# ysymyth/3D-SDN

Hardware: AMD Instinct MI355X
Metric: rendered-objects/sec (FFD decode + transform + silhouette/normal/depth @384, fwd+bwd) (higher is better)
Workload: dtype f32

## Files before the change

3d-sdn_amd/csrc/fast_ffd.hip:

```cpp
#include "sdn_common.h"

namespace sdn {

constexpr int NCOEF_MAX = 512;

__global__ __launch_bounds__(256) void k_ffd_fwd(const float* __restrict__ Bt, const float* __restrict__ P,
                                                  const int32_t* __restrict__ cls, int vmax, int ncoef,
                                                  float* __restrict__ out)
{
    __shared__ float Ps[3 * NCOEF_MAX];
    const int b = blockIdx.y;
    for (int t = threadIdx.x; t < 3 * ncoef; t += 256) Ps[t] = P[(size_t)b * 3 * ncoef + t];
    __syncthreads();
    const int v = blockIdx.x * 256 + threadIdx.x;
    if (v >= vmax) return;
    const float* bt = Bt + (size_t)cls[b] * ncoef * vmax + v;
    float x = 0.f, y = 0.f, z = 0.f;
#pragma unroll 8
    for (int j = 0; j < ncoef; j++) {
        const float w = bt[(size_t)j * vmax];
        x += Ps[j] * w;
        y += Ps[ncoef + j] * w;
        z += Ps[2 * ncoef + j] * w;
    }
// ... 21 lines not shown
        const float g0 = gb[3 * v + 0], g1 = gb[3 * v + 1], g2 = gb[3 * v + 2];
#pragma unroll
        for (int u = 0; u < FFD_JB; u++) {
            const float w = (j0 + u < ncoef) ? bt[(size_t)u * vmax + v] : 0.f;
            s[u][0] += g0 * w;
            s[u][1] += g1 * w;
            s[u][2] += g2 * w;
        }
    }
#pragma unroll
    for (int u = 0; u < FFD_JB; u++) {
#pragma unroll
        for (int o = 32; o > 0; o >>= 1) {
            s[u][0] += __shfl_xor(s[u][0], o, 64);
            s[u][1] += __shfl_xor(s[u][1], o, 64);
            s[u][2] += __shfl_xor(s[u][2], o, 64);
        }
        if ((threadIdx.x & 63) == 0) {
            red[u][0][threadIdx.x >> 6] = s[u][0];
            red[u][1][threadIdx.x >> 6] = s[u][1];
            red[u][2][threadIdx.x >> 6] = s[u][2];
        }
    }
    __syncthreads();
    if (threadIdx.x < 3 * FFD_JB) {
        const int u = threadIdx.x / 3, d = threadIdx.x % 3;
        if (j0 + u < ncoef) {
            float t = 0.f;
#pragma unroll
            for (int w = 0; w < NW; w++) t += red[u][d][w];
            grad_P[((size_t)b * 3 + d) * ncoef + j0 + u] = t;
        }
    }
}

__global__ __launch_bounds__(256) void k_ffd_coefficients(const float* __restrict__ x, const float* __restrict__ M,
                                                          const float* __restrict__ base, int m, int transpose,
                                                          float* __restrict__ out)
{
    extern __shared__ float xrow[];
    float* part = xrow + m;
    const int i = blockIdx.y;
    for (int k = threadIdx.x; k < m; k += 256) xrow[k] = x[(size_t)i * m + k];
    __syncthreads();
    const int jj = threadIdx.x & 63, kq = threadIdx.x >> 6;
    const int j = blockIdx.x * 64 + jj;
    const int per = (m + 3) / 4, k0 = kq * per, k1 = min(m, k0 + per);
    float acc = 0.0f;
    if (j < m) {
        if (transpose) {
            const float* row = M + (size_t)j * m;
#pragma unroll 8
            for (int k = k0; k < k1; k++) acc = fmaf(xrow[k], row[k], acc);
        } else {
#pragma unroll 8
            for (int k = k0; k < k1; k++) acc = fmaf(xrow[k], M[(size_t)k * m + j], acc);
        }
    }
    part[kq * 64 + jj] = acc;
    __syncthreads();
    if (kq == 0 && j < m)
        out[(size_t)i * m + j] = (base ? base[j] : 0.0f) + ((part[jj] + part[64 + jj]) + (part[128 + jj] + part[192 + jj]));
}

}

using namespace sdn;

SDN_API int sdn_ffd_coefficients(const float* x, const float* M, const float* base, int n, int m, int transpose, float* out,
                                 sdnStream stream)
{
    if (!x || !M || !out || n <= 0 || m <= 0 || m > 12288)
        return fail(SDN_EINVAL, "sdn_ffd_coefficients: bad arguments (m <= 12288)");
    hipLaunchKernelGGL(k_ffd_coefficients, dim3(cdiv(m, 64), n), dim3(256), (size_t)(m + 256) * sizeof(float), (hipStream_t)stream,
                       x, M, base, m, transpose, out);
    return check_launch("k_ffd_coefficients");
}

SDN_API int sdn_ffd_decode(const float* Bt, const float* P, const int32_t* cls, int n, int vmax, int ncoef, float* out,
                           sdnStream stream)
{
    if (!Bt || !P || !cls || !out || n <= 0 || vmax <= 0 || ncoef <= 0 || ncoef > NCOEF_MAX)
        return fail(SDN_EINVAL, "sdn_ffd_decode: bad arguments (ncoef <= %d)", NCOEF_MAX);
    hipLaunchKernelGGL(k_ffd_fwd, dim3(cdiv(vmax, 256), n), dim3(256), 0, (hipStream_t)stream, Bt, P, cls, vmax, ncoef,
                       out);
    return check_launch("k_ffd_fwd");
}

SDN_API int sdn_ffd_decode_bwd(const float* Bt, const int32_t* cls, const float* grad_out, int n, int vmax, int ncoef,
                               float* grad_P, sdnStream stream)
{
    if (!Bt || !cls || !grad_out || !grad_P || n <= 0 || vmax <= 0 || ncoef <= 0 || ncoef > NCOEF_MAX)
        return fail(SDN_EINVAL, "sdn_ffd_decode_bwd: bad arguments");
    hipLaunchKernelGGL(k_ffd_bwd, dim3(cdiv(ncoef, FFD_JB), n), dim3(FFD_BWD_THREADS), 0, (hipStream_t)stream, Bt, cls, grad_out, vmax, ncoef,
                       grad_P);
    return check_launch("k_ffd_bwd");
}
```

3d-sdn_amd/geometric/derender3d/models/transforms.py:

```python
import numpy as np
import scipy.special
import torch

from torch.nn.modules import Module


class _Constraint(object):

    class Type:
        symmetry = 0
        homogeneity = 1

    class Axis:
        x = 0
        y = 1
        z = 2

    def __init__(self, type, axis=None, index=None):
        self.type = type
        self.axis = axis
        self.index = index

    @classmethod
    def symmetry(cls, axis):
# ... 25 lines not shown
            shape = [1] * dP.dim()
            shape[comp] = 3
            dP = dP.index_copy(ax, idx, torch.where(keep.reshape(shape), planes, mean))
    return dP


def bernstein_basis(t, one_minus_t, n):
    i = torch.arange(n, dtype=torch.float32)
    binom = torch.tensor(scipy.special.binom(n - 1, np.arange(n)), dtype=torch.float32)
    return binom * torch.pow(t[:, None], i) * torch.pow(one_minus_t[:, None], n - 1 - i)


class FFD(Module):

    Constraint = _Constraint

    @staticmethod
    def flip(x, dim):
        return torch.flip(x, dims=(dim,))

    def __init__(self, vertices, num_grids=4, constraints=None):
        super(FFD, self).__init__()
        if num_grids % 2:
            raise AssertionError('num_grids must be even')
        self.num_grids = num_grids
        self.constraints = list(constraints) if constraints is not None else []
        v = torch.as_tensor(vertices, dtype=torch.float32)
        per_axis = [bernstein_basis(0.5 + v[:, d], 0.5 - v[:, d], num_grids) for d in range(3)]
        B = torch.einsum('ni,nj,nk->nijk', per_axis[0], per_axis[1], per_axis[2])
        lattice = torch.linspace(0, num_grids - 1, num_grids)
        P0 = torch.stack(torch.meshgrid(lattice, lattice, lattice, indexing='ij')) / (num_grids - 1) - 0.5
        self.register_buffer('B', B[:, None], persistent=False)
        self.register_buffer('P0', P0, persistent=False)

    def constrain(self, ffd_coeff):
        g = self.num_grids
        return apply_constraints(ffd_coeff.reshape(3, g, g, g), self.constraints)

    def forward(self, ffd_coeff):
        dP = self.constrain(ffd_coeff)
        n3 = self.num_grids ** 3
        P = (self.P0.to(dP.device) + dP).reshape(3, n3)
        return torch.matmul(self.B.to(dP.device).reshape(-1, n3), P.t())


def constrain_batched(dP, constraints, num_grids):
    return apply_constraints(dP, constraints)


class FFDBank(Module):

    def __init__(self, ffds, faces_list):
        super(FFDBank, self).__init__()
        from sdn_hip import ops
        self.num_grids = ffds[0].num_grids
        self.constraints = ffds[0].constraints
        n3 = self.num_grids ** 3
        self.nverts = [int(f.B.shape[0]) for f in ffds]
        self.nfaces = [int(f.shape[0]) for f in faces_list]
        vmax, fmax = max(self.nverts), max(self.nfaces)
        Bt = torch.zeros(len(ffds), n3, vmax)
        faces = torch.zeros(len(ffds), fmax, 3, dtype=torch.int32)
        for c, (ffd, f) in enumerate(zip(ffds, faces_list)):
            B = ffd.B.reshape(-1, n3)
            Bt[c, :, :B.shape[0]] = B.t()
            Bt[c, :, B.shape[0]:] = B[0][:, None]
            faces[c, :f.shape[0]] = f
        self.register_buffer('Bt', Bt.contiguous(), persistent=False)
        self.register_buffer('faces', faces.contiguous(), persistent=False)
        self.register_buffer('P0', ffds[0].P0.reshape(3, n3).clone(), persistent=False)
        eye = torch.eye(3 * n3).reshape(3 * n3, 3, self.num_grids, self.num_grids, self.num_grids)
        C = constrain_batched(eye, self.constraints, self.num_grids).reshape(3 * n3, 3 * n3)
        self.register_buffer('constraint_matrix', C.contiguous(), persistent=False)

    def decode(self, ffd_coeffs, classes):
        from sdn_hip import ops
        n = ffd_coeffs.shape[0]
        g = self.num_grids
        cls, faces = self._class_rows(classes)
        verts = ops.FFDDecode.apply(ffd_coeffs.reshape(n, 3 * g ** 3), self.Bt, cls, self.constraint_matrix, self.P0)
        return verts, faces

    def _class_rows(self, classes):
        hit = self.__dict__.get('_rows_cache')
        if hit is not None and hit[0] is classes and hit[1] == classes._version:
            return hit[2], hit[3]
        cls = classes.to(torch.int32)
        faces = self.faces.index_select(0, classes.long())
        self.__dict__['_rows_cache'] = (classes, classes._version, cls, faces)
        return cls, faces


    def invalidate_class_cache(self):
        self.__dict__.pop('_rows_cache', None)


class PerspectiveTransform(Module):
    def forward(self,
                vertices,
                scales=None,
                rotations=None,
                translations=None,
                perspective_translations=None,
                zooms=None,
                zoom_tos=None):
        if (vertices.is_cuda and scales is not None and rotations is not None and translations is not None
                and (zoom_tos is None) != (zooms is None) and vertices.dim() == 3):
            from sdn_hip import ops
            n = vertices.shape[0]
            persp = translations if perspective_translations is None else perspective_translations

            def full(x, k):
                return x.reshape(-1, k).expand(n, k) if x.shape[0] != n else x.reshape(n, k)
            t3 = full(translations, 3)
# ... 37 lines not shown
```

3d-sdn_amd/sdn_hip/__init__.py:

```python
import ctypes
import os
import threading

import torch

_HERE = os.path.dirname(os.path.abspath(__file__))
LIB_PATH = os.path.normpath(os.path.join(_HERE, '..', 'lib', 'libsdn_hip.so'))

RGB, ALPHA, DEPTH, AA, FACE_COLOR, SAVE_MAPS, ACCUMULATE, SERIAL_EDGES, STREAM_FACES, COUNT_WORK = 1, 2, 4, 8, 16, 32, 64, 128, 256, 512
K1_COVERAGE = 4096

ABI_VERSION = 20

_lib = None
_lock = threading.Lock()
_vp = ctypes.c_void_p
_ci = ctypes.c_int
_cl = ctypes.c_long
_cd = ctypes.c_double
_sz = ctypes.c_size_t


class SdnHipError(RuntimeError):
    pass


def _declare(L):
    L.sdn_last_error.restype = ctypes.c_char_p
    L.sdn_version.restype = _ci
    sig = {
        'sdn_project_vertices': [_vp, _ci, _ci, _ci, _vp, _vp, _vp, _vp, _ci, _vp, _vp],
        'sdn_project_vertices_bwd': [_vp, _ci, _ci, _ci, _vp, _vp, _vp, _vp, _ci, _vp, _vp, _vp],
        'sdn_gather_faces': [_vp, _vp, _ci, _ci, _ci, _cl, _ci, _vp, _vp],
        'sdn_gather_faces_bwd': [_vp, _vp, _ci, _ci, _ci, _cl, _ci, _vp, _vp],
        'sdn_face_normals': [_vp, _cl, _vp, _vp],
        'sdn_face_normals_bwd': [_vp, _vp, _cl, _vp, _vp],
        'sdn_raster_workspace_bytes': [_ci, _ci, _ci, ctypes.POINTER(_sz)],
        'sdn_rasterize_fwd': [_vp, _vp, _ci, _ci, _ci, _ci, _cd, _cd, _cd, _vp, _ci, _ci, _vp, _vp, _vp, _vp, _vp,
                              _vp, _vp, _vp, _vp, _sz, _vp],
        'sdn_raster_bwd_workspace_bytes': [_ci, _ci, _ci, ctypes.POINTER(_sz)],
        'sdn_rasterize_bwd': [_vp, _vp, _ci, _ci, _ci, _ci, _cd, _ci, _vp, _vp, _vp, _vp, _vp, _vp, _vp, _vp, _vp,
                              _vp, _vp, _sz, _vp],
    }
    sig['sdn_raster_work_counters'] = [_vp, _ci, _ci, _ci, ctypes.POINTER(ctypes.c_ulonglong), _vp]
    sig['sdn_ffd_decode'] = [_vp, _vp, _vp, _ci, _ci, _ci, _vp, _vp]
    sig['sdn_ffd_decode_bwd'] = [_vp, _vp, _vp, _ci, _ci, _ci, _vp, _vp]
    _i8p = ctypes.POINTER(ctypes.c_int8)
    _cf = ctypes.c_float
    sig['sdn_conv_gemm_workspace_bytes'] = [_ci, _ci, _ci, _ci, ctypes.POINTER(_sz)]
    sig['sdn_conv_gemm'] = [_vp, _ci, _ci, _ci, _ci, _vp, _ci, _ci, _ci, _ci, _ci, _ci, _ci, _ci, _ci, _ci, _i8p, _i8p,
                            _ci, _ci, _vp, _ci, _ci, _vp, _ci, _vp, _ci, _ci, _vp, _sz, _vp]
    _i32p = ctypes.POINTER(ctypes.c_int32)
    sig['sdn_conv_gemm_phases'] = [_vp, _ci, _ci, _ci, _ci, _vp, _ci, _ci, _ci, _ci, _ci, _ci, _i32p, _i32p, _i32p, _i32p, _i32p, _i8p,
                                   _ci, _ci, ctypes.POINTER(_vp), _i32p, _ci, _vp, _ci, _vp, _ci, _ci, _vp]
    sig['sdn_conv_wgrad'] = [_vp, _vp, _vp, _ci, _ci, _ci, _ci, _ci, _ci, _ci, _ci, _ci, _i8p, _i8p, _ci, _ci, _ci, _ci,
                             _ci, _vp, _sz, _vp]
    sig['sdn_conv_wgrad_narrow'] = [_vp, _vp, _vp, _ci, _ci, _ci, _ci, _ci, _ci, _ci, _ci, _ci, _i8p, _i8p, _ci, _ci, _ci,
                                    _vp]
    sig['sdn_conv_wgrad_head_mfma'] = [_vp, _vp, _vp, _ci, _ci, _ci, _ci, _ci, _ci, _ci, _ci, _ci, _i8p, _i8p, _ci, _ci, _ci,
                                    _vp]
    sig['sdn_conv_narrow_fwd'] = [_vp, _ci, _ci, _ci, _ci, _vp, _ci, _ci, _ci, _ci, _vp, _ci, _ci, _ci, _ci, _ci, _ci,
                                  _vp, _ci, _vp]
    sig['sdn_conv_head_steps'] = [_ci, _ci, _ci, ctypes.POINTER(_ci)]
    sig['sdn_conv_head_mfma'] = [_vp, _ci, _ci, _ci, _ci, _vp, _ci, _ci, _ci, _ci, _vp, _ci, _ci, _ci, _ci, _ci, _ci, _vp, _ci, _vp, _vp]
    sig['sdn_in_apply'] = [_vp, _vp, _vp, _vp, _vp, _ci, _ci, _ci, _ci, _cf, _ci, _ci, _cf, _vp, _vp, _vp, _cl, _ci, _vp]
    sig['sdn_in_bwd'] = [_vp, _vp, _vp, _vp, _ci, _ci, _ci, _ci, _vp, _cl, _vp]
    sig['sdn_act_bwd'] = [_vp, _vp, _vp, _cl, _ci, _ci, _vp, _cl, _vp]
    sig['sdn_reflect_fold'] = [_vp, _vp, _ci, _ci, _ci, _ci, _ci, _ci, _vp]
    sig['sdn_conv_pack_weights'] = [_vp, _ci, _ci, _cl, _cl, _vp, _ci, _ci, _ci, _ci, _vp, _vp]
    sig['sdn_conv_unpack_grad'] = [_vp, _ci, _ci, _cl, _cl, _vp, _ci, _ci, _vp, _ci, _vp]
    sig['sdn_split_planes'] = [_vp, _cl, _ci, _vp, _cl, _vp]
    sig['sdn_assemble_nhwc'] = [_vp, _vp, _ci, _ci, _ci, _ci, _ci, _vp, _vp]
    sig['sdn_conv_pack_weights_kmajor'] = [_vp, _ci, _ci, _cl, _cl, _vp, _ci, _ci, _ci, _vp, _vp]
    sig['sdn_conv_tile'] = [_vp, _cl, _ci, _ci, _ci, _ci, _vp, _vp, _cl, _ci, _ci, _ci, _ci, _ci, _ci, _ci, _ci, _ci, _ci, _ci,
                            _i8p, _i8p, _ci, _vp, _ci, _vp, _ci, _vp, _ci, _ci, _vp]
    sig['sdn_conv_halo_blocks'] = [_ci, _ci, _ci, _ci, _ci, _ci, ctypes.POINTER(_ci), ctypes.POINTER(_ci), ctypes.POINTER(_cl)]
    sig['sdn_conv_halo'] = [_vp, _cl, _ci, _ci, _ci, _ci, _vp, _ci, _ci, _ci, _ci, _i8p, _i8p, _ci, _vp, _ci, _vp, _ci, _vp, _ci, _vp]
    sig['sdn_conv_wgrad_tile'] = [_vp, _cl, _vp, _cl, _vp, _ci, _ci, _ci, _ci, _ci, _ci, _ci, _ci, _ci, _i8p, _i8p, _ci, _vp]
    sig['sdn_segment_mean'] = [_vp, _vp, _ci, _ci, _ci, _ci, _vp, _vp, _vp, _vp]
# ... 91 lines not shown
    for name, argtypes in sig.items():
        try:
            fn = getattr(L, name)
        except AttributeError:
            raise SdnHipError('%s does not export %s -- rebuild it (`python __graft_entry__.py build`)' % (LIB_PATH, name))
        fn.argtypes = argtypes
        fn.restype = _ci
    return sig


def lib():
    global _lib
    if _lib is None:
        with _lock:
            if _lib is None:
                if not os.path.exists(LIB_PATH):
                    raise SdnHipError(
                        'libsdn_hip.so not found at %s -- run `python __graft_entry__.py build` (hipcc, gfx950); '
                        'there is no CPU or PyTorch fallback for this path' % LIB_PATH)
                L = ctypes.CDLL(LIB_PATH)
                L.sdn_version.restype = _ci
                have = L.sdn_version()
                if have != ABI_VERSION:
                    raise SdnHipError('%s reports ABI version %d, this binding needs %d -- rebuild it '
                                      '(`python __graft_entry__.py build`)' % (LIB_PATH, have, ABI_VERSION))
                _declare(L)
                _lib = L
    return _lib


def exported_symbols():
    return ['sdn_last_error', 'sdn_version', 'sdn_project_vertices', 'sdn_project_vertices_bwd', 'sdn_gather_faces',
            'sdn_gather_faces_bwd', 'sdn_face_normals', 'sdn_face_normals_bwd', 'sdn_raster_workspace_bytes',
            'sdn_rasterize_fwd', 'sdn_raster_work_counters', 'sdn_raster_bwd_workspace_bytes', 'sdn_rasterize_bwd', 'sdn_ffd_decode', 'sdn_ffd_decode_bwd', 'sdn_ffd_coefficients',
            'sdn_timing_enable', 'sdn_timing_declare_work', 'sdn_timing_read', 'sdn_timing_read_slot', 'sdn_conv_gemm', 'sdn_conv_gemm_phases', 'sdn_conv_gemm_workspace_bytes', 'sdn_conv_wgrad', 'sdn_conv_wgrad_narrow', 'sdn_conv_wgrad_head_mfma', 'sdn_conv_narrow_fwd', 'sdn_conv_head_steps', 'sdn_conv_head_mfma', 'sdn_in_apply', 'sdn_in_bwd',
            'sdn_act_bwd', 'sdn_reflect_fold', 'sdn_conv_pack_weights', 'sdn_conv_unpack_grad', 'sdn_split_planes', 'sdn_conv_pack_weights_kmajor',
            'sdn_conv_tile', 'sdn_conv_wgrad_tile', 'sdn_conv_halo', 'sdn_conv_halo_blocks', 'sdn_segment_mean', 'sdn_l1_loss_fwd', 'sdn_l1_loss_bwd', 'sdn_silhouette_loss_fwd', 'sdn_silhouette_loss_bwd', 'sdn_assemble_nhwc', 'sdn_pose_params', 'sdn_pose_algebra', 'sdn_pose_algebra_bwd',
            'sdn_pose_params_bwd', 'sdn_composite_frame', 'sdn_edit_assemble', 'sdn_scene_cover', 'sdn_scene_crops', 'sdn_scene_edit',
            'sdn_unmold_masks', 'sdn_scene_gt_masks', 'sdn_scene_paint2d',
            'sdn_scene_id_workspace_bytes', 'sdn_scene_id_stats', 'sdn_scene_id_planes', 'sdn_assemble_planes', 'sdn_assemble_maps',
            'sdn_train_rois', 'sdn_train_crops', 'sdn_train_id_stats_workspace_bytes', 'sdn_train_id_stats', 'sdn_train_crops_mixed',
            'sdn_train_losses_scratch', 'sdn_train_losses_fwd', 'sdn_train_losses_bwd',
            'sdn_segm_fuse', 'sdn_segm_labels_from_colors', 'sdn_segm_confusion', 'sdn_segm_train_batch', 'sdn_segm_loss_fwd', 'sdn_segm_loss_bwd',
            'sdn_segm_ppm_pool', 'sdn_segm_ppm_fill', 'sdn_segm_ppm_fill_bwd', 'sdn_segm_ppm_pool_bwd',
            'sdn_encode_maps', 'sdn_inst_index_workspace_bytes', 'sdn_inst_index_build', 'sdn_inst_index_rank',
            'sdn_mrcnn_loss_workspace_bytes', 'sdn_mrcnn_loss_fwd', 'sdn_mrcnn_loss_bwd',
            'sdn_pyramid_roi_align_grad_floats', 'sdn_pyramid_roi_align_fwd', 'sdn_pyramid_roi_align_bwd',
            'sdn_proposal_layer_workspace_bytes', 'sdn_proposal_layer',
            'sdn_detection_layer_workspace_bytes', 'sdn_detection_layer',
            'sdn_detection_targets_workspace_bytes', 'sdn_detection_targets',
            'sdn_rpn_targets_workspace_bytes', 'sdn_rpn_targets',
            'sdn_perspective_transform_scratch', 'sdn_perspective_transform', 'sdn_perspective_transform_bwd', 'sdn_bn_forward', 'sdn_bn_backward',
            'sdn_maxpool3x3s2_fwd', 'sdn_maxpool3x3s2_bwd', 'sdn_avgpool_global', 'sdn_nms_workspace_bytes', 'sdn_nms',
            'sdn_crop_and_resize_fwd', 'sdn_crop_and_resize_bwd', 'sdn_avgpool3x3s2_fwd', 'sdn_avgpool3x3s2_bwd', 'sdn_render_maps_bytes', 'sdn_render_maps_fwd', 'sdn_raster_phase_clocks',
            'sdn_render_maps_bwd', 'sdn_program_create', 'sdn_program_run',
            'sdn_program_destroy']


def check(rc):
    if rc != 0:
        raise SdnHipError('libsdn_hip error %d: %s' % (rc, lib().sdn_last_error().decode()))


def ptr(t):
    return None if t is None else t.data_ptr()


# ... 10 lines not shown
        raise NotImplementedError('%s is on %s; this renderer only runs on the GPU' % (name, t.device))
    if t.dtype != dtype:
        raise TypeError('%s must be %s, got %s' % (name, dtype, t.dtype))
    return t.contiguous()


_const_cache = {}


def const_f32(values, device):
    import numpy as np
    a = np.ascontiguousarray(np.asarray(values, dtype=np.float32))
    key = (a.tobytes(), a.shape, str(device))
    t = _const_cache.get(key)
    if t is None:
        if len(_const_cache) > 4096:
            _const_cache.clear()
        t = _const_cache[key] = torch.tensor(a, device=device)
    return t


def raster_workspace(bs, nf, S, device):
    n = _sz(0)
    check(lib().sdn_raster_workspace_bytes(bs, nf, S, ctypes.byref(n)))
    return torch.empty(n.value, dtype=torch.uint8, device=device)


def perspective_transform_scratch(n, V):
    kb, ab = _sz(0), _sz(0)
    check(lib().sdn_perspective_transform_scratch(n, V, ctypes.byref(kb), ctypes.byref(ab)))
    return kb.value, ab.value


def train_losses_scratch(B, R, nffd):
    n = _sz(0)
    check(lib().sdn_train_losses_scratch(B, R, nffd, ctypes.byref(n)))
    return n.value


def raster_bwd_workspace(bs, nf, S, device):
    n = _sz(0)
    check(lib().sdn_raster_bwd_workspace_bytes(bs, nf, S, ctypes.byref(n)))
    return torch.empty(n.value, dtype=torch.uint8, device=device)


def scene_id_workspace(device):
    n = _sz(0)
    check(lib().sdn_scene_id_workspace_bytes(ctypes.byref(n)))
    return torch.empty(n.value, dtype=torch.uint8, device=device)


def train_id_workspace(B, device):
    n = _sz(0)
    check(lib().sdn_train_id_stats_workspace_bytes(int(B), ctypes.byref(n)))
    return torch.empty(n.value, dtype=torch.uint8, device=device)


def timing_enable(on=True):
    check(lib().sdn_timing_enable(int(bool(on))))


def timing_read():
    ms, n = _cd(0), _cl(0)
    check(lib().sdn_timing_read(ctypes.byref(ms), ctypes.byref(n)))
    return ms.value, n.value

# ... 10 lines not shown
```

3d-sdn_amd/sdn_hip/ops.py:

```python
import ctypes

import numpy as np
import torch
from torch.autograd.function import once_differentiable

from . import (AA, ACCUMULATE, ALPHA, COUNT_WORK, DEPTH, FACE_COLOR, K1_COVERAGE, RGB, SAVE_MAPS, SERIAL_EDGES, STREAM_FACES, check, lib, ptr, raster_bwd_workspace,
               raster_workspace, scene_id_workspace, stream, train_id_workspace, want)

CAMERA_NONE, CAMERA_LOOK, CAMERA_LOOK_AT = 0, 1, 2

import threading

_tls = threading.local()


class verification:

    def __init__(self, serial_edges=None, stream_faces=None, count_work=None):
        new = dict(serial_edges=serial_edges, stream_faces=stream_faces, count_work=count_work)
        self.new = {k: v for k, v in new.items() if v is not None}

    def __enter__(self):
        self.old = {k: getattr(_tls, k, False) for k in self.new}
        for k, v in self.new.items():
# ... 21 lines not shown
    return _K1[0]


def last_clocks():
    return getattr(_tls, 'last_clocks', None)


def last_work():
    return getattr(_tls, 'last_work', None)


def perspective_width(angle):
    a = np.float32(angle)
    a = np.float32(a / np.float32(180.))
    a = np.float32(a * np.float32(3.1416))
    return np.float32(np.tan(a, dtype=np.float32))


def _f32(t, name):
    return want(t, torch.float32, name)


_ptf_sizes = {}


def _ptf_scratch(n, V):
    r = _ptf_sizes.get((n, V))
    if r is None:
        from . import perspective_transform_scratch
        if len(_ptf_sizes) > 256:
            _ptf_sizes.clear()
        r = _ptf_sizes[(n, V)] = perspective_transform_scratch(n, V)
    return r


class ProjectVertices(torch.autograd.Function):
    @staticmethod
    def forward(ctx, vertices, camera_mode, eye, direction, up, width, flip_x):
        v = _f32(vertices, 'vertices')
        if v.dim() != 3 or v.shape[2] != 3:
            raise ValueError('vertices must be [batch, n, 3]')
        bs, nv = v.shape[:2]
        eye = _f32(eye, 'eye')
        direction = _f32(direction, 'direction')
        up = _f32(up, 'up')
        width = _f32(width, 'width')
        for t, n in ((eye, 'eye'), (direction, 'direction'), (up, 'up')):
            if t is not None and tuple(t.shape) != (bs, 3):
                raise ValueError('%s must be [batch, 3]' % n)
        if width is not None and width.numel() != bs:
            raise ValueError('width must have one entry per batch element')
        out = torch.empty_like(v)
        check(lib().sdn_project_vertices(ptr(v), bs, nv, int(camera_mode), ptr(eye), ptr(direction), ptr(up),
                                         ptr(width), int(flip_x), ptr(out), stream()))
        ctx.save_for_backward(v, eye, direction, up, width)
        ctx.cfg = (int(camera_mode), int(flip_x))
        return out

    @staticmethod
    def backward(ctx, g):
        v, eye, direction, up, width = ctx.saved_tensors
        mode, flip_x = ctx.cfg
        g = g.contiguous()
        gv = torch.empty_like(v)
        bs, nv = v.shape[:2]
        check(lib().sdn_project_vertices_bwd(ptr(v), bs, nv, mode, ptr(eye), ptr(direction), ptr(up), ptr(width),
# ... 225 lines not shown
                ctx.save_for_backward(v, f, state, cam[1], cam[2], cam[3], cam[4], bg)
                ctx.bg = None
            else:
                ctx.save_for_backward(v, f, state, cam[1], cam[2], cam[3], cam[4])
                ctx.bg = bg
            ctx.cfg = (bs, nv, nf0, stride, int(bool(fill_back)), cam[0], cam[5], R, flags & ~STREAM_FACES, float(eps),
                       float(eps_alpha), nbwd.value, SERIAL_EDGES if _switch('serial_edges') else 0)
        ctx.set_materialize_grads(False)
        return alpha, normal, depth

    @staticmethod
    def backward(ctx, g_alpha, g_normal, g_depth):
        saved = ctx.saved_tensors
        v, f, state, eye, direction, up, width = saved[:7]
        bg = saved[7] if len(saved) > 7 else ctx.bg
        bs, nv, nf0, stride, fill_back, mode, flip_x, R, flags, eps, eps_alpha, nbwd, serial = ctx.cfg
        if g_alpha is None and g_normal is None and g_depth is None:
            return (None,) * 18
        g_alpha = None if g_alpha is None else g_alpha.contiguous()
        g_normal = None if g_normal is None else g_normal.contiguous()
        g_depth = None if g_depth is None else g_depth.contiguous()
        ws = torch.empty(nbwd, dtype=torch.uint8, device=v.device)
        gv = torch.empty_like(v)
        check(lib().sdn_render_maps_bwd(ptr(v), bs, nv, ptr(f), nf0, stride, fill_back, mode, ptr(eye), ptr(direction), ptr(up),
                                        ptr(width), flip_x, R, flags | serial, eps, eps_alpha, ptr(bg), ptr(g_alpha),
                                        ptr(g_normal), ptr(g_depth), ptr(gv), ptr(state), state.numel(), ptr(ws), ws.numel(),
                                        stream()))
        return (gv,) + (None,) * 17


class FFDDecode(torch.autograd.Function):

    @staticmethod
    def forward(ctx, P, Bt, cls, constraint=None, base=None):
        P = _f32(P, 'P')
        Bt = _f32(Bt, 'Bt')
        cls = want(cls, torch.int32, 'cls')
        n = P.shape[0]
        ncoef = Bt.shape[1] if Bt.dim() == 3 else -1
        if constraint is not None:
            Cm = _f32(constraint, 'constraint')
            m = 3 * ncoef
            if P.dim() != 2 or P.shape[1] != m or tuple(Cm.shape) != (m, m) or (base is not None and base.numel() != m):
                raise ValueError('FFDDecode: coefficients [n, 3 ncoef], constraint [3 ncoef, 3 ncoef], base [3, ncoef]')
            base = None if base is None else _f32(base, 'base')
            coeffs = P
            P = torch.empty((n, 3, ncoef), dtype=torch.float32, device=coeffs.device)
            check(lib().sdn_ffd_coefficients(ptr(coeffs), ptr(Cm), ptr(base), n, m, 0, ptr(P), stream()))
        else:
            Cm = None
        if P.dim() != 3 or P.shape[1] != 3 or Bt.dim() != 3 or P.shape[2] != ncoef or cls.numel() != n:
            raise ValueError('FFDDecode: P [n,3,ncoef], Bt [classes,ncoef,vmax], cls [n]')
        vmax = Bt.shape[2]
        out = torch.empty((n, vmax, 3), dtype=torch.float32, device=P.device)
        check(lib().sdn_ffd_decode(ptr(Bt), ptr(P), ptr(cls), n, vmax, ncoef, ptr(out), stream()))
        if Cm is None:
            ctx.save_for_backward(Bt, cls)
        else:
            ctx.save_for_backward(Bt, cls, Cm)
        ctx.cfg = (n, vmax, ncoef)
        return out

    @staticmethod
    def backward(ctx, g):
        Bt, cls = ctx.saved_tensors[:2]
        n, vmax, ncoef = ctx.cfg
        g = g.contiguous()
        gP = torch.empty((n, 3, ncoef), dtype=torch.float32, device=g.device)
        check(lib().sdn_ffd_decode_bwd(ptr(Bt), ptr(cls), ptr(g), n, vmax, ncoef, ptr(gP), stream()))
        if len(ctx.saved_tensors) == 3:
            gc = torch.empty((n, 3 * ncoef), dtype=torch.float32, device=g.device)
            check(lib().sdn_ffd_coefficients(ptr(gP), ptr(ctx.saved_tensors[2]), None, n, 3 * ncoef, 1, ptr(gc), stream()))
            return gc, None, None, None, None
        return gP, None, None, None, None


class PoseParamsFn(torch.autograd.Function):

    @staticmethod
    def forward(ctx, theta, log_scales):
        th = _f32(theta, 'theta').reshape(-1)
        n = th.shape[0]
        ls = _f32(log_scales, 'log_scales').reshape(n, 3)
        quat = torch.empty(n, 4, dtype=torch.float32, device=th.device)
        scales = torch.empty(n, 3, dtype=torch.float32, device=th.device)
        check(lib().sdn_pose_params(ptr(th), ptr(ls), n, ptr(quat), ptr(scales), stream()))
        ctx.save_for_backward(th, scales)
        ctx.shapes = (theta.shape, log_scales.shape)
        ctx.set_materialize_grads(False)
        return quat, scales

    @staticmethod
    def backward(ctx, g_quat, g_scales):
        th, scales = ctx.saved_tensors
        n = th.shape[0]
        want_t, want_s = ctx.needs_input_grad
        if g_quat is None and g_scales is None:
            return None, None
        gq = g_quat.contiguous() if g_quat is not None else None
        gs = g_scales.contiguous() if g_scales is not None else None
        gt = torch.empty(n, dtype=torch.float32, device=th.device) if want_t else None
        gl = torch.empty(n, 3, dtype=torch.float32, device=th.device) if want_s else None
        if gt is None and gl is None:
            return None, None
        check(lib().sdn_pose_params_bwd(ptr(th), ptr(scales), ptr(gq), ptr(gs), n, ptr(gt), ptr(gl), stream()))
        return (gt.reshape(ctx.shapes[0]) if gt is not None else None, gl.reshape(ctx.shapes[1]) if gl is not None else None)

# ... 1665 lines not shown
```

include/sdn_hip.h:

```cpp
#ifndef SDN_HIP_H
#define SDN_HIP_H

#include <stddef.h>
#include <stdint.h>

#ifdef __cplusplus
extern "C" {
#endif

typedef void* sdnStream;

#define SDN_OK 0
#define SDN_EINVAL (-1)
#define SDN_ELAUNCH (-2)
#define SDN_ENOMEM (-3)

#define SDN_RGB 1
#define SDN_ALPHA 2
#define SDN_DEPTH 4
#define SDN_AA 8
#define SDN_FACE_COLOR 16
#define SDN_SAVE_MAPS 32
#define SDN_ACCUMULATE 64
#define SDN_STREAM_FACES 256
// ... 27 lines not shown

int sdn_rasterize_fwd(const float* faces, const float* textures, int ts, int bs, int nf, int S,
                      double near, double far, double eps, const float* bg, int bg_per_batch, int flags,
                      float* face_inv, int32_t* face_index_map, float* weight_map, float* depth_map,
                      float* rgb_map, float* rgb_out, float* alpha_out, float* depth_out,
                      void* workspace, size_t workspace_bytes, sdnStream stream);

int sdn_raster_work_counters(const void* workspace, int bs, int nf, int S, unsigned long long* out3, sdnStream stream);

int sdn_raster_phase_clocks(const void* workspace, int bs, int nf, int S, unsigned long long* out8, sdnStream stream);

int sdn_raster_bwd_workspace_bytes(int bs, int nf, int S, size_t* out);
int sdn_rasterize_bwd(const float* faces, const float* textures, int ts, int bs, int nf, int S,
                      double eps, int flags, const float* face_inv, const int32_t* face_index_map,
                      const float* weight_map, const float* depth_map, const float* rgb_map,
                      const float* g_rgb_out, const float* g_alpha_out, const float* g_depth_out,
                      float* grad_faces, float* grad_textures, void* workspace, size_t workspace_bytes,
                      sdnStream stream);

int sdn_render_maps_bytes(int bs, int nv, int nf0, int fill_back, int image_size, int flags, size_t* state_bytes,
                          size_t* bwd_workspace_bytes, size_t* fwd_scratch_bytes);
int sdn_render_maps_fwd(const float* verts, int bs, int nv, const int32_t* faces_idx, int nf0, long faces_batch_stride,
                        int fill_back, int camera_mode, const float* eye, const float* dir, const float* up,
                        const float* width, int flip_x, int image_size, int flags, double near, double far, double eps,
                        const float* bg, float* alpha_out, float* normal_out, float* depth_out, void* state,
                        size_t state_bytes, void* scratch, size_t scratch_bytes, sdnStream stream);
int sdn_render_maps_bwd(const float* verts, int bs, int nv, const int32_t* faces_idx, int nf0, long faces_batch_stride,
                        int fill_back, int camera_mode, const float* eye, const float* dir, const float* up,
                        const float* width, int flip_x, int image_size, int flags, double eps, double eps_alpha,
                        const float* bg, const float* g_alpha, const float* g_normal, const float* g_depth, float* grad_verts,
                        const void* state, size_t state_bytes, void* workspace, size_t workspace_bytes, sdnStream stream);

int sdn_ffd_decode(const float* Bt, const float* P, const int32_t* cls, int n, int vmax, int ncoef,
                   float* out, sdnStream stream);
int sdn_ffd_decode_bwd(const float* Bt, const int32_t* cls, const float* grad_out, int n, int vmax,
                       int ncoef, float* grad_P, sdnStream stream);
int sdn_ffd_coefficients(const float* x, const float* M, const float* base, int n, int m, int transpose, float* out,
                         sdnStream stream);


#define SDN_STAT_SLOTS 8
int sdn_conv_gemm_workspace_bytes(int N, int OH, int OW, int Cop, size_t* out);
int sdn_conv_gemm(const float* in, int N, int IH, int IW, int Cip, float* out, int OH, int OW, int Cop, int QH, int QW,
                  int istride, int ostride, int py, int px, int ntaps, const int8_t* dy, const int8_t* dx, int pad_mode,
                  int in_relu, const void* w_packed, int Kp, int w_rows, const float* bias, int act,
                  double* stats, int accumulate, int precision, void* workspace, size_t workspace_bytes,
                  sdnStream stream);

int sdn_conv_gemm_phases(const float* in, int N, int IH, int IW, int Cip, float* out, int OH, int OW, int Cop, int istride,
                         int ostride, int nphase, const int32_t* QH, const int32_t* QW, const int32_t* py, const int32_t* px,
                         const int32_t* ntaps, const int8_t* taps, int pad_mode, int in_relu, const void* const* w_packed,
                         const int32_t* Kp, int w_rows, const float* bias, int act, double* stats, int accumulate,
                         int precision, sdnStream stream);

int sdn_conv_wgrad(const float* rows, const float* gath, float* dw, int N, int QH, int QW, int Cr, int GH, int GW, int Cc,
                   int istride, int ntaps, const int8_t* dy, const int8_t* dx, int pad_mode, int relu_rows,
                   int relu_gath, int splits, int precision, void* workspace, size_t workspace_bytes, sdnStream stream);
int sdn_conv_wgrad_narrow(const float* rows, const float* gath, float* dw, int N, int QH, int QW, int Cr, int rows_used,
                          int GH, int GW, int Cc, int ntaps, const int8_t* dy, const int8_t* dx, int pad_mode,
                          int relu_rows, int relu_gath, sdnStream stream);

int sdn_conv_wgrad_head_mfma(const float* rows, const float* gath, float* dw, int N, int QH, int QW, int Cr, int rows_used,
                             int GH, int GW, int Cc, int ntaps, const int8_t* dy, const int8_t* dx, int pad_mode,
                             int relu_rows, int relu_gath, sdnStream stream);

int sdn_conv_narrow_fwd(const float* in, int N, int IH, int IW, int Cip, float* out, int QH, int QW, int Cop,
                        int rows_used, const float* w_dense, int KH, int KW, int dy_min, int dx_min, int pad_mode,
                        int in_relu, const float* bias, int act, sdnStream stream);

// ... 295 lines not shown
```

Baseline: 24440.

## Decode FFD from per-axis Bernstein factors and use MFMA in backward

Stores the 4x4x4 FFD basis as three per-axis factor tables (12 rows per vertex instead of 64). The forward pass rebuilds the 64 weights on the fly as products, with contraction disabled so it matches the stored table bitwise. The backward pass stages gradients and factors in shared memory and accumulates the 3x64 outer products with 16x16x4 fp32 MFMA over chunks of vertices. Partial sums go to a workspace and are reduced by a last-block ticket. This cuts the basis-table memory traffic, at the cost of a workspace, atomics, and a path that only applies when the factorization check passes.

Result: slower. 23230 (-5.0%).

```diff
diff --git a/3d-sdn_amd/csrc/fast_ffd.hip b/3d-sdn_amd/csrc/fast_ffd.hip
--- a/3d-sdn_amd/csrc/fast_ffd.hip
+++ b/3d-sdn_amd/csrc/fast_ffd.hip
@@ -77,6 +77,145 @@
             grad_P[((size_t)b * 3 + d) * ncoef + j0 + u] = t;
         }
     }
+}
+
+constexpr int FFD_G = 4, FFD_G3 = 64;
+
+__device__ __forceinline__ float ffd_mul(float a, float b)
+{
+#pragma clang fp contract(off) reassociate(off)
+    return a * b;
+}
+
+__global__ __launch_bounds__(256) void k_ffd_factored_fwd(const float* __restrict__ F, const float* __restrict__ P,
+                                                           const int32_t* __restrict__ cls, int vmax, float* __restrict__ out)
+{
+    const int b = blockIdx.y;
+    const float* __restrict__ p = P + (size_t)b * 3 * FFD_G3;
+    const int v = blockIdx.x * 256 + threadIdx.x;
+    if (v >= vmax) return;
+    const float* f = F + (size_t)cls[b] * 3 * FFD_G * vmax + v;
+    float fx[FFD_G], fy[FFD_G], fz[FFD_G];
+#pragma unroll
+    for (int i = 0; i < FFD_G; i++) {
+        fx[i] = f[(size_t)i * vmax];
+        fy[i] = f[(size_t)(FFD_G + i) * vmax];
+        fz[i] = f[(size_t)(2 * FFD_G + i) * vmax];
+    }
+    float x = 0.f, y = 0.f, z = 0.f;
+#pragma unroll
+    for (int i = 0; i < FFD_G; i++) {
+#pragma unroll
+        for (int jj = 0; jj < FFD_G; jj++) {
+            const float t = ffd_mul(fx[i], fy[jj]);
+#pragma unroll
+            for (int k = 0; k < FFD_G; k++) {
+                const int j = (i * FFD_G + jj) * FFD_G + k;
+                const float w = ffd_mul(t, fz[k]);
+                x += p[j] * w;
+                y += p[FFD_G3 + j] * w;
+                z += p[2 * FFD_G3 + j] * w;
+            }
+        }
+    }
+    float* o = out + ((size_t)b * vmax + v) * 3;
+    o[0] = x;
+    o[1] = y;
+    o[2] = z;
+}
+
+constexpr int FFD_FB_VERTS = 1024, FFD_FB_THREADS = 512, FFD_FB_PITCH = FFD_FB_VERTS + 16, FFD_FB_ROWS = 15, FFD_SUM_BATCH = 8;
+constexpr size_t FFD_TICKET_ALIGN = 256;
+typedef float ffd_f32x4 __attribute__((ext_vector_type(4)));
+
+__global__ __launch_bounds__(FFD_FB_THREADS) void k_ffd_factored_bwd(const float* __restrict__ F, const int32_t* __restrict__ cls,
+                                                                      const float* __restrict__ g, int vmax, int nchunks,
+                                                                      float* part, int* tickets, float* grad_P)
+{
+    constexpr int NW = FFD_FB_THREADS / 64, PER_WAVE = FFD_FB_VERTS / NW, PER_THREAD = FFD_FB_VERTS / FFD_FB_THREADS;
+    static_assert(PER_WAVE == 128 && PER_THREAD * FFD_FB_THREADS == FFD_FB_VERTS, "8 groups of 16 vertices per wave");
+    __shared__ __attribute__((aligned(16))) float slab[FFD_FB_ROWS * FFD_FB_PITCH];
+    float (*red)[3 * FFD_G3] = reinterpret_cast<float (*)[3 * FFD_G3]>(slab);
+    static_assert(NW * 3 * FFD_G3 <= FFD_FB_ROWS * FFD_FB_PITCH, "the waves' tiles fit the slab");
+    const int b = blockIdx.y, chunk = blockIdx.x, tid = threadIdx.x;
+    const int v0 = chunk * FFD_FB_VERTS, nv = min(FFD_FB_VERTS, vmax - v0);
+    const float* gb = g + ((size_t)b * vmax + v0) * 3;
+    const float* f = F + (size_t)cls[b] * 3 * FFD_G * vmax + v0;
+    float gv[3 * PER_THREAD], fv[3 * FFD_G][PER_THREAD];
+#pragma unroll
+    for (int u = 0; u < 3 * PER_THREAD; u++) gv[u] = gb[min(tid + u * FFD_FB_THREADS, 3 * nv - 1)];
+#pragma unroll
+    for (int r = 0; r < 3 * FFD_G; r++)
+#pragma unroll
+        for (int u = 0; u < PER_THREAD; u++) fv[r][u] = f[(size_t)r * vmax + min(tid + u * FFD_FB_THREADS, nv - 1)];
+#pragma unroll
+    for (int u = 0; u < 3 * PER_THREAD; u++) {
+        const int e = tid + u * FFD_FB_THREADS;
+        slab[(e % 3) * FFD_FB_PITCH + e / 3] = e < 3 * nv ? gv[u] : 0.f;
+    }
+#pragma unroll
+    for (int r = 0; r < 3 * FFD_G; r++)
+#pragma unroll
+        for (int u = 0; u < PER_THREAD; u++) {
+            const int v = tid + u * FFD_FB_THREADS;
+            slab[(3 + r) * FFD_FB_PITCH + v] = v < nv ? fv[r][u] : 0.f;
+        }
+    __syncthreads();
+    const int wave = tid >> 6, lane = tid & 63, r = lane & 15, q = lane >> 4;
+    const bool live = r < 3 * FFD_G;
+    const float* sg = slab + min(r >> 2, 2) * FFD_FB_PITCH;
+    const float* sx = slab + (3 + (r & 3)) * FFD_FB_PITCH;
+    const float* sy = slab + (3 + FFD_G + (r >> 2)) * FFD_FB_PITCH;
+    const float* sz = slab + (3 + 2 * FFD_G + (r & 3)) * FFD_FB_PITCH;
+    ffd_f32x4 acc0 = {0.f, 0.f, 0.f, 0.f}, acc1 = {0.f, 0.f, 0.f, 0.f};
+    const int first = wave * PER_WAVE;
+    if (first < nv) {
+#pragma unroll
+        for (int t = 0; t < PER_WAVE / 16; t++) {
+            const int at = first + t * 16 + q * 4;
+            const ffd_f32x4 G = *reinterpret_cast<const ffd_f32x4*>(sg + at), X = *reinterpret_cast<const ffd_f32x4*>(sx + at);
+            const ffd_f32x4 Y = *reinterpret_cast<const ffd_f32x4*>(sy + at), Z = *reinterpret_cast<const ffd_f32x4*>(sz + at);
+            acc0 = __builtin_amdgcn_mfma_f32_16x16x4f32(live ? G.x * X.x : 0.f, Y.x * Z.x, acc0, 0, 0, 0);
+            acc1 = __builtin_amdgcn_mfma_f32_16x16x4f32(live ? G.y * X.y : 0.f, Y.y * Z.y, acc1, 0, 0, 0);
+            acc0 = __builtin_amdgcn_mfma_f32_16x16x4f32(live ? G.z * X.z : 0.f, Y.z * Z.z, acc0, 0, 0, 0);
+            acc1 = __builtin_amdgcn_mfma_f32_16x16x4f32(live ? G.w * X.w : 0.f, Y.w * Z.w, acc1, 0, 0, 0);
+        }
+    }
+    __syncthreads();
+    if (q < 3) {
+        red[wave][q * FFD_G3 + 0 * 16 + r] = acc0.x + acc1.x;
+        red[wave][q * FFD_G3 + 1 * 16 + r] = acc0.y + acc1.y;
+        red[wave][q * FFD_G3 + 2 * 16 + r] = acc0.z + acc1.z;
+        red[wave][q * FFD_G3 + 3 * 16 + r] = acc0.w + acc1.w;
+    }
+    __syncthreads();
+    if (tid < 3 * FFD_G3) {
+        float s = red[0][tid];
+#pragma unroll
+        for (int w = 1; w < NW; w++) s += red[w][tid];
+        part[((size_t)b * nchunks + chunk) * 3 * FFD_G3 + tid] = s;
+    }
+    if (nchunks == 1) return;
+    __shared__ int last;
+    __threadfence();
+    __syncthreads();
+    if (tid == 0) last = atomicAdd(tickets + b, 1) == nchunks - 1;
+    __syncthreads();
+    if (!last) return;
+    __threadfence();
+    if (tid < 3 * FFD_G3) {
+        const float* p = part + (size_t)b * nchunks * 3 * FFD_G3 + tid;
+        float s = 0.f;
+        for (int c0 = 0; c0 < nchunks; c0 += FFD_SUM_BATCH) {
+            float a[FFD_SUM_BATCH];
+#pragma unroll
+            for (int u = 0; u < FFD_SUM_BATCH; u++) a[u] = p[(size_t)min(c0 + u, nchunks - 1) * 3 * FFD_G3];
+#pragma unroll
+            for (int u = 0; u < FFD_SUM_BATCH; u++) s += c0 + u < nchunks ? a[u] : 0.f;
+        }
+        grad_P[(size_t)b * 3 * FFD_G3 + tid] = s;
+    }
+    if (tid == 0) tickets[b] = 0;
 }
 
 __global__ __launch_bounds__(256) void k_ffd_coefficients(const float* __restrict__ x, const float* __restrict__ M,
@@ -122,21 +261,46 @@
     return check_launch("k_ffd_coefficients");
 }
 
-SDN_API int sdn_ffd_decode(const float* Bt, const float* P, const int32_t* cls, int n, int vmax, int ncoef, float* out,
-                           sdnStream stream)
-{
-    if (!Bt || !P || !cls || !out || n <= 0 || vmax <= 0 || ncoef <= 0 || ncoef > NCOEF_MAX)
+SDN_API int sdn_ffd_decode(const float* Bt, const float* P, const int32_t* cls, int n, int vmax, int ncoef,
+                           const float* factors, float* out, sdnStream stream)
+{
+    if ((!Bt && !factors) || !P || !cls || !out || n <= 0 || vmax <= 0 || ncoef <= 0 || ncoef > NCOEF_MAX)
         return fail(SDN_EINVAL, "sdn_ffd_decode: bad arguments (ncoef <= %d)", NCOEF_MAX);
+    if (factors) {
+        if (ncoef != FFD_G3 || n > 65535) return fail(SDN_EINVAL, "sdn_ffd_decode: factors are for ncoef == %d, n <= 65535", FFD_G3);
+        hipLaunchKernelGGL(k_ffd_factored_fwd, dim3(cdiv(vmax, 256), n), dim3(256), 0, (hipStream_t)stream, factors, P, cls, vmax,
+                           out);
+        return check_launch("k_ffd_factored_fwd");
+    }
     hipLaunchKernelGGL(k_ffd_fwd, dim3(cdiv(vmax, 256), n), dim3(256), 0, (hipStream_t)stream, Bt, P, cls, vmax, ncoef,
                        out);
     return check_launch("k_ffd_fwd");
 }
 
+SDN_API int sdn_ffd_decode_bwd_workspace_bytes(int n, int vmax, size_t* out)
+{
+    if (!out || n <= 0 || vmax <= 0) return fail(SDN_EINVAL, "sdn_ffd_decode_bwd_workspace_bytes: bad arguments");
+    *out = (size_t)cdiv((size_t)n * sizeof(int), FFD_TICKET_ALIGN) * FFD_TICKET_ALIGN +
+           (size_t)n * cdiv(vmax, FFD_FB_VERTS) * 3 * FFD_G3 * sizeof(float);
+    return SDN_OK;
+}
+
 SDN_API int sdn_ffd_decode_bwd(const float* Bt, const int32_t* cls, const float* grad_out, int n, int vmax, int ncoef,
-                               float* grad_P, sdnStream stream)
-{
-    if (!Bt || !cls || !grad_out || !grad_P || n <= 0 || vmax <= 0 || ncoef <= 0 || ncoef > NCOEF_MAX)
+                               const float* factors, float* grad_P, void* workspace, size_t workspace_bytes, sdnStream stream)
+{
+    if ((!Bt && !factors) || !cls || !grad_out || !grad_P || n <= 0 || vmax <= 0 || ncoef <= 0 || ncoef > NCOEF_MAX)
         return fail(SDN_EINVAL, "sdn_ffd_decode_bwd: bad arguments");
+    if (factors) {
+        const int nchunks = (int)cdiv(vmax, FFD_FB_VERTS);
+        if (ncoef != FFD_G3 || n > 65535) return fail(SDN_EINVAL, "sdn_ffd_decode_bwd: factors are for ncoef == %d, n <= 65535", FFD_G3);
+        const size_t head = (size_t)cdiv((size_t)n * sizeof(int), FFD_TICKET_ALIGN) * FFD_TICKET_ALIGN;
+        if (nchunks > 1 && (!workspace || workspace_bytes < head + (size_t)n * nchunks * 3 * FFD_G3 * sizeof(float)))
+            return fail(SDN_EINVAL, "sdn_ffd_decode_bwd: workspace too small (sdn_ffd_decode_bwd_workspace_bytes)");
+        float* part = nchunks > 1 ? (float*)((char*)workspace + head) : grad_P;
+        hipLaunchKernelGGL(k_ffd_factored_bwd, dim3(nchunks, n), dim3(FFD_FB_THREADS), 0, (hipStream_t)stream, factors, cls, grad_out,
+                           vmax, nchunks, part, (int*)workspace, grad_P);
+        return check_launch("k_ffd_factored_bwd");
+    }
     hipLaunchKernelGGL(k_ffd_bwd, dim3(cdiv(ncoef, FFD_JB), n), dim3(FFD_BWD_THREADS), 0, (hipStream_t)stream, Bt, cls, grad_out, vmax, ncoef,
                        grad_P);
     return check_launch("k_ffd_bwd");
diff --git a/3d-sdn_amd/geometric/derender3d/models/transforms.py b/3d-sdn_amd/geometric/derender3d/models/transforms.py
--- a/3d-sdn_amd/geometric/derender3d/models/transforms.py
+++ b/3d-sdn_amd/geometric/derender3d/models/transforms.py
@@ -81,6 +81,8 @@
         P0 = torch.stack(torch.meshgrid(lattice, lattice, lattice, indexing='ij')) / (num_grids - 1) - 0.5
         self.register_buffer('B', B[:, None], persistent=False)
         self.register_buffer('P0', P0, persistent=False)
+        for name, table in zip(('Bx', 'By', 'Bz'), per_axis):
+            self.register_buffer(name, table, persistent=False)
 
     def constrain(self, ffd_coeff):
         g = self.num_grids
@@ -116,6 +118,7 @@
             Bt[c, :, B.shape[0]:] = B[0][:, None]
             faces[c, :f.shape[0]] = f
         self.register_buffer('Bt', Bt.contiguous(), persistent=False)
+        self.register_buffer('F', self._factor_table(ffds, vmax), persistent=False)
         self.register_buffer('faces', faces.contiguous(), persistent=False)
         self.register_buffer('P0', ffds[0].P0.reshape(3, n3).clone(), persistent=False)
         eye = torch.eye(3 * n3).reshape(3 * n3, 3, self.num_grids, self.num_grids, self.num_grids)
@@ -127,8 +130,27 @@
         n = ffd_coeffs.shape[0]
         g = self.num_grids
         cls, faces = self._class_rows(classes)
-        verts = ops.FFDDecode.apply(ffd_coeffs.reshape(n, 3 * g ** 3), self.Bt, cls, self.constraint_matrix, self.P0)
+        verts = ops.FFDDecode.apply(ffd_coeffs.reshape(n, 3 * g ** 3), self.Bt, cls, self.constraint_matrix, self.P0, self.F)
         return verts, faces
+
+    @staticmethod
+    def _factor_table(ffds, vmax):
+        if ffds[0].num_grids != 4:
+            return None
+        F = torch.zeros(len(ffds), 12, vmax)
+        for c, ffd in enumerate(ffds):
+            tables = [getattr(ffd, name, None) for name in ('Bx', 'By', 'Bz')]
+            B = ffd.B.reshape(-1, 4, 4, 4)
+            if any(t is None or t.dtype != torch.float32 or tuple(t.shape) != (B.shape[0], 4) for t in tables) or B.dtype != torch.float32:
+                return None
+            bx, by, bz = (t.to(B.device) for t in tables)
+            product = (bx[:, :, None, None] * by[:, None, :, None]) * bz[:, None, None, :]
+            if not torch.equal(product.contiguous().view(torch.int32), B.contiguous().view(torch.int32)):
+                return None
+            rows = torch.cat((bx, by, bz), dim=1).t().cpu()
+            F[c, :, :rows.shape[1]] = rows
+            F[c, :, rows.shape[1]:] = rows[:, :1]
+        return F.contiguous()
 
     def _class_rows(self, classes):
         hit = self.__dict__.get('_rows_cache')
diff --git a/3d-sdn_amd/sdn_hip/__init__.py b/3d-sdn_amd/sdn_hip/__init__.py
--- a/3d-sdn_amd/sdn_hip/__init__.py
+++ b/3d-sdn_amd/sdn_hip/__init__.py
@@ -43,8 +43,9 @@
                               _vp, _vp, _sz, _vp],
     }
     sig['sdn_raster_work_counters'] = [_vp, _ci, _ci, _ci, ctypes.POINTER(ctypes.c_ulonglong), _vp]
-    sig['sdn_ffd_decode'] = [_vp, _vp, _vp, _ci, _ci, _ci, _vp, _vp]
-    sig['sdn_ffd_decode_bwd'] = [_vp, _vp, _vp, _ci, _ci, _ci, _vp, _vp]
+    sig['sdn_ffd_decode'] = [_vp, _vp, _vp, _ci, _ci, _ci, _vp, _vp, _vp]
+    sig['sdn_ffd_decode_bwd_workspace_bytes'] = [_ci, _ci, ctypes.POINTER(_sz)]
+    sig['sdn_ffd_decode_bwd'] = [_vp, _vp, _vp, _ci, _ci, _ci, _vp, _vp, _vp, _sz, _vp]
     _i8p = ctypes.POINTER(ctypes.c_int8)
     _cf = ctypes.c_float
     sig['sdn_conv_gemm_workspace_bytes'] = [_ci, _ci, _ci, _ci, ctypes.POINTER(_sz)]
@@ -202,7 +203,7 @@
 def exported_symbols():
     return ['sdn_last_error', 'sdn_version', 'sdn_project_vertices', 'sdn_project_vertices_bwd', 'sdn_gather_faces',
             'sdn_gather_faces_bwd', 'sdn_face_normals', 'sdn_face_normals_bwd', 'sdn_raster_workspace_bytes',
-            'sdn_rasterize_fwd', 'sdn_raster_work_counters', 'sdn_raster_bwd_workspace_bytes', 'sdn_rasterize_bwd', 'sdn_ffd_decode', 'sdn_ffd_decode_bwd', 'sdn_ffd_coefficients',
+            'sdn_rasterize_fwd', 'sdn_raster_work_counters', 'sdn_raster_bwd_workspace_bytes', 'sdn_rasterize_bwd', 'sdn_ffd_decode', 'sdn_ffd_decode_bwd_workspace_bytes', 'sdn_ffd_decode_bwd', 'sdn_ffd_coefficients',
             'sdn_timing_enable', 'sdn_timing_declare_work', 'sdn_timing_read', 'sdn_timing_read_slot', 'sdn_conv_gemm', 'sdn_conv_gemm_phases', 'sdn_conv_gemm_workspace_bytes', 'sdn_conv_wgrad', 'sdn_conv_wgrad_narrow', 'sdn_conv_wgrad_head_mfma', 'sdn_conv_narrow_fwd', 'sdn_conv_head_steps', 'sdn_conv_head_mfma', 'sdn_in_apply', 'sdn_in_bwd',
             'sdn_act_bwd', 'sdn_reflect_fold', 'sdn_conv_pack_weights', 'sdn_conv_unpack_grad', 'sdn_split_planes', 'sdn_conv_pack_weights_kmajor',
             'sdn_conv_tile', 'sdn_conv_wgrad_tile', 'sdn_conv_halo', 'sdn_conv_halo_blocks', 'sdn_segment_mean', 'sdn_l1_loss_fwd', 'sdn_l1_loss_bwd', 'sdn_silhouette_loss_fwd', 'sdn_silhouette_loss_bwd', 'sdn_assemble_nhwc', 'sdn_pose_params', 'sdn_pose_algebra', 'sdn_pose_algebra_bwd',
@@ -279,6 +280,12 @@
     return kb.value, ab.value
 
 
+def ffd_decode_bwd_workspace_bytes(n, vmax):
+    nb = _sz(0)
+    check(lib().sdn_ffd_decode_bwd_workspace_bytes(n, vmax, ctypes.byref(nb)))
+    return nb.value
+
+
 def train_losses_scratch(B, R, nffd):
     n = _sz(0)
     check(lib().sdn_train_losses_scratch(B, R, nffd, ctypes.byref(n)))
diff --git a/3d-sdn_amd/sdn_hip/ops.py b/3d-sdn_amd/sdn_hip/ops.py
--- a/3d-sdn_amd/sdn_hip/ops.py
+++ b/3d-sdn_amd/sdn_hip/ops.py
@@ -77,6 +77,23 @@
             _ptf_sizes.clear()
         r = _ptf_sizes[(n, V)] = perspective_transform_scratch(n, V)
     return r
+
+
+_ffd_bwd_ws = {}
+
+
+def _ffd_bwd_workspace(device, n, vmax):
+    key = (device, n, vmax)
+    ws = _ffd_bwd_ws.get(key)
+    if ws is None:
+        from . import ffd_decode_bwd_workspace_bytes
+        nb = ffd_decode_bwd_workspace_bytes(n, vmax)
+        ws = torch.zeros(nb, dtype=torch.uint8, device=device)
+        if nb:
+            if len(_ffd_bwd_ws) > 64:
+                _ffd_bwd_ws.clear()
+            _ffd_bwd_ws[key] = ws
+    return ws
 
 
 class ProjectVertices(torch.autograd.Function):
@@ -368,12 +385,16 @@
 class FFDDecode(torch.autograd.Function):
 
     @staticmethod
-    def forward(ctx, P, Bt, cls, constraint=None, base=None):
+    def forward(ctx, P, Bt, cls, constraint=None, base=None, factors=None):
         P = _f32(P, 'P')
         Bt = _f32(Bt, 'Bt')
         cls = want(cls, torch.int32, 'cls')
         n = P.shape[0]
         ncoef = Bt.shape[1] if Bt.dim() == 3 else -1
+        if factors is not None:
+            factors = _f32(factors, 'factors')
+            if Bt.dim() != 3 or ncoef != 64 or tuple(factors.shape) != (Bt.shape[0], 12, Bt.shape[2]):
+                raise ValueError('FFDDecode: factors [classes, 12, vmax] go with Bt [classes, 64, vmax]')
         if constraint is not None:
             Cm = _f32(constraint, 'constraint')
             m = 3 * ncoef
@@ -389,26 +410,25 @@
             raise ValueError('FFDDecode: P [n,3,ncoef], Bt [classes,ncoef,vmax], cls [n]')
         vmax = Bt.shape[2]
         out = torch.empty((n, vmax, 3), dtype=torch.float32, device=P.device)
-        check(lib().sdn_ffd_decode(ptr(Bt), ptr(P), ptr(cls), n, vmax, ncoef, ptr(out), stream()))
-        if Cm is None:
-            ctx.save_for_backward(Bt, cls)
-        else:
-            ctx.save_for_backward(Bt, cls, Cm)
+        check(lib().sdn_ffd_decode(ptr(Bt), ptr(P), ptr(cls), n, vmax, ncoef, ptr(factors), ptr(out), stream()))
+        ctx.save_for_backward(Bt, cls, Cm, factors)
         ctx.cfg = (n, vmax, ncoef)
         return out
 
     @staticmethod
     def backward(ctx, g):
-        Bt, cls = ctx.saved_tensors[:2]
+        Bt, cls, Cm, factors = ctx.saved_tensors
         n, vmax, ncoef = ctx.cfg
         g = g.contiguous()
         gP = torch.empty((n, 3, ncoef), dtype=torch.float32, device=g.device)
-        check(lib().sdn_ffd_decode_bwd(ptr(Bt), ptr(cls), ptr(g), n, vmax, ncoef, ptr(gP), stream()))
-        if len(ctx.saved_tensors) == 3:
+        ws = None if factors is None else _ffd_bwd_workspace(g.device, n, vmax)
+        check(lib().sdn_ffd_decode_bwd(ptr(Bt), ptr(cls), ptr(g), n, vmax, ncoef, ptr(factors), ptr(gP), ptr(ws),
+                                       0 if ws is None else ws.numel(), stream()))
+        if Cm is not None:
             gc = torch.empty((n, 3 * ncoef), dtype=torch.float32, device=g.device)
-            check(lib().sdn_ffd_coefficients(ptr(gP), ptr(ctx.saved_tensors[2]), None, n, 3 * ncoef, 1, ptr(gc), stream()))
-            return gc, None, None, None, None
-        return gP, None, None, None, None
+            check(lib().sdn_ffd_coefficients(ptr(gP), ptr(Cm), None, n, 3 * ncoef, 1, ptr(gc), stream()))
+            return gc, None, None, None, None, None
+        return gP, None, None, None, None, None
 
 
 class PoseParamsFn(torch.autograd.Function):
diff --git a/include/sdn_hip.h b/include/sdn_hip.h
--- a/include/sdn_hip.h
+++ b/include/sdn_hip.h
@@ -83,9 +83,11 @@
                         const void* state, size_t state_bytes, void* workspace, size_t workspace_bytes, sdnStream stream);
 
 int sdn_ffd_decode(const float* Bt, const float* P, const int32_t* cls, int n, int vmax, int ncoef,
-                   float* out, sdnStream stream);
+                   const float* factors, float* out, sdnStream stream);
+int sdn_ffd_decode_bwd_workspace_bytes(int n, int vmax, size_t* out);
 int sdn_ffd_decode_bwd(const float* Bt, const int32_t* cls, const float* grad_out, int n, int vmax,
-                       int ncoef, float* grad_P, sdnStream stream);
+                       int ncoef, const float* factors, float* grad_P, void* workspace, size_t workspace_bytes,
+                       sdnStream stream);
 int sdn_ffd_coefficients(const float* x, const float* M, const float* base, int n, int m, int transpose, float* out,
                          sdnStream stream);
 
```
